# mfathulkr/MA-CJD-Cooperative-Jamming-Decision-Making-via-MARL

Measured on AMD Instinct MI355X. Metric: env-steps/sec (all GPUs; batch_envs=4096/GPU, 3j/4r), higher is better.
Workload: dtype f64; 1 GPU; 3 jammers / 4 radars, batch_envs=4096 per GPU, GRU hidden=64; mode=train, hidden=64, train_batch_episodes=32, updates_per_graph=20, hip_graphs=True, gemm_tuning=True, replay_capacity_episodes=8192, mixer_dtype=fp32, mixer=one MFMA launch per direction (f32)

## Files before the change

### include/macjd_nets.h

```cpp
#ifndef MACJD_NETS_H
#define MACJD_NETS_H

#include <stdint.h>

#include "macjd.h"

#ifdef __cplusplus
extern "C" {
#endif

typedef struct macjd_qhead_io {
    int64_t n_rows;
    int32_t H, A, n_agents, greedy_only;
    const float* base;  int64_t base_ld;
    const float* P_all; int64_t p_ld;
    const float* W1;    int64_t w1_ld;
    const float* w2;
    const float* b2;
    float* Q;           int64_t q_ld;
    const void* avail;  int32_t avail_elem_size, reserved;
    int64_t av_se, av_sj, av_sa;
    float epsilon;      float reserved2;
    uint64_t seed, counter;
    const float* eps_dev;
// ... 106 lines not shown
typedef struct macjd_wgrad_norm_io {
    int32_t ln_problem, partials_cap;
    const float* W; int64_t w_ld;
    float* dgamma; float* dbeta;
    float* partials;
    float* step;
} macjd_wgrad_norm_io;

int32_t macjd_linear_wgrad_many_norm_partials(const macjd_wgrad_io* ios, int32_t n, int32_t ln_problem);
int macjd_linear_wgrad_many_norm(const macjd_wgrad_io* ios, int32_t n, const macjd_wgrad_norm_io* norm, void* hip_stream);

int macjd_clip_adam_step_reduced(const macjd_adam_io* io, int32_t n_partials, const macjd_sampler_io* next, void* hip_stream);

typedef struct macjd_gather_io {
    int32_t n_tensors, n_rows;
    const int64_t* idx;
    const void* src[8]; void* dst[8]; int64_t row_bytes[8];
    int64_t dst_row_bytes[8];
} macjd_gather_io;

int macjd_gather_rows(const macjd_gather_io* io, void* hip_stream);

typedef struct macjd_prefetch_io {
    macjd_gru_io gru;
    macjd_gather_io gather;
    macjd_sampler_io sampler;
    macjd_tdloss_io mask;
    float* tot_m;
    int32_t no_draw, gather_blocks;
} macjd_prefetch_io;

int macjd_prefetch_batch_supported(int32_t n_nets, int32_t H, int32_t B);
int macjd_prefetch_batch(const macjd_prefetch_io* io, void* hip_stream);

typedef struct macjd_qinput_io {
    int64_t n_rows;
    int32_t H, A;
    const float* h;   int64_t h_ld;
    const void* idx;  int32_t idx_elem_size, reserved;
    const float* P;
    float* out;       int64_t out_ld;
} macjd_qinput_io;

int macjd_qhead_input(const macjd_qinput_io* io, void* hip_stream);

typedef struct macjd_qtaken_io {
    int64_t n_rows;
    int32_t H, A;
    const float* h;   int64_t h_ld;
    const void* idx;  int32_t idx_elem_size, reserved;
    const float* P;
    const float* W1;  int64_t w1_ld;
    const float* b1;  const float* w2;  const float* b2;
    float* x;         int64_t x_ld;
    float* act;       int64_t act_ld;
    float* q;
} macjd_qtaken_io;

int macjd_qhead_taken_supported(int32_t H, int32_t A);
int macjd_qhead_taken(const macjd_qtaken_io* io, void* hip_stream);

typedef struct macjd_layernorm_io {
    int64_t M;
    int32_t S, reserved;
    float eps, reserved2;
    const float* x;  int64_t x_ld;
// ... 238 lines not shown
```

### ma-cjd-cooperative-jamming-decision-making-via-marl_amd/_native.py

```python
from __future__ import annotations

import ctypes
import os
from typing import Optional

_PKG_DIR = os.path.dirname(os.path.abspath(__file__))
LIB_NAME = "libmacjd_hip.so"
LIB_PATH = os.environ.get("MACJD_LIB") or os.path.join(_PKG_DIR, LIB_NAME)

ABI_VERSION = 9
STEP_ARITH_F64 = 1
STEP_LANE_KERNEL = 2
STEP_SLOT_KERNEL = 4

EXPORTS = [
    "macjd_abi_version", "macjd_last_error", "macjd_reload_options", "macjd_device_count",
    "macjd_scenario_create", "macjd_scenario_destroy", "macjd_scenario_dims", "macjd_scenario_is_regular",
    "macjd_env_reset", "macjd_env_step", "macjd_env_step_timed",
    "macjd_qhead_select", "macjd_gru_sequence", "macjd_mixer_tail_forward", "macjd_mixer_tail_backward",
    "macjd_mlp_forward", "macjd_mlp_forward_pair", "macjd_td_loss", "macjd_clip_adam_step", "macjd_clip_adam_step_sample", "macjd_clip_adam_step_ln", "macjd_sample_episodes", "macjd_gather_rows",
    "macjd_linear_wgrad", "macjd_linear_wgrad_workspace_floats", "macjd_linear_wgrad_many", "macjd_qhead_input", "macjd_layernorm_forward", "macjd_layernorm_param_grad", "macjd_gru_gates", "macjd_rowdot", "macjd_splitrelu_backward",
    "macjd_mixer_fused_supported", "macjd_mixer_fused_forward", "macjd_mixer_fused_backward", "macjd_mixer_fused_backward_td", "macjd_td_mask_sum",
    "macjd_agent_episode_supported", "macjd_agent_episode", "macjd_env_step_many", "macjd_env_step_many_timed",
    "macjd_qhead_double_q_supported", "macjd_qhead_double_q", "macjd_qhead_taken_supported", "macjd_qhead_taken",
    "macjd_qheads_pair", "macjd_mixer_fused_forward_pair", "macjd_mixer_fused_train", "macjd_mixer_fused_train_static",
    "macjd_scenario_set_scan", "macjd_env_step_scan", "macjd_env_reset_scan",
    "macjd_env_step_scan_pe", "macjd_env_reset_scan_pe",
    "macjd_agent_env_episode_scan_supported", "macjd_agent_env_episode_scan",
    "macjd_scenario_set_scan_pattern",
    "macjd_gru_sequence_backward_supported", "macjd_gru_sequence_backward",
    "macjd_prefetch_batch_supported", "macjd_prefetch_batch",
    "macjd_actor_gradient_supported", "macjd_actor_gradient",
    "macjd_linear_wgrad_many_norm", "macjd_linear_wgrad_many_norm_partials", "macjd_clip_adam_step_reduced",
]


class NativeLibraryError(RuntimeError):
    pass


class StepIO(ctypes.Structure):
    _fields_ = [
        ("n_envs", ctypes.c_int64), ("env_offset", ctypes.c_int64), ("seed", ctypes.c_uint64),
        ("flags", ctypes.c_uint32), ("reserved", ctypes.c_uint32),
        ("T", ctypes.c_void_p), ("T_se", ctypes.c_int64), ("T_sx", ctypes.c_int64),
        ("P32", ctypes.c_void_p), ("P64", ctypes.c_void_p), ("P_se", ctypes.c_int64), ("P_sx", ctypes.c_int64),
        ("u", ctypes.c_void_p), ("u_se", ctypes.c_int64), ("u_sx", ctypes.c_int64),
        ("episode", ctypes.c_void_p),
        ("track", ctypes.c_void_p), ("k_se", ctypes.c_int64), ("k_sx", ctypes.c_int64),
        ("step", ctypes.c_void_p),
        ("reward", ctypes.c_void_p), ("r_dpj", ctypes.c_void_p), ("terminated", ctypes.c_void_p),
        ("pd", ctypes.c_void_p), ("pd_se", ctypes.c_int64), ("pd_sx", ctypes.c_int64),
        ("snr_with", ctypes.c_void_p), ("sw_se", ctypes.c_int64), ("sw_sx", ctypes.c_int64),
        ("out64", ctypes.c_void_p), ("pd64", ctypes.c_void_p), ("snr64", ctypes.c_void_p),
        ("prj64", ctypes.c_void_p),
        ("pe_tables", ctypes.c_void_p), ("pe_flags", ctypes.c_void_p), ("pe_stride", ctypes.c_int64),
        ("pe_tile", ctypes.c_int32), ("reserved_pe", ctypes.c_int32),
        ("r_dpj_sum", ctypes.c_void_p),
    ]


class ScanDesc(ctypes.Structure):
    _fields_ = [
        ("n_radars", ctypes.c_int32), ("n_jammers", ctypes.c_int32),
        ("half_beam", ctypes.c_void_p), ("sweep", ctypes.c_void_p), ("sweep_mod", ctypes.c_void_p),
        ("full", ctypes.c_void_p), ("az0", ctypes.c_void_p), ("bear_tgt", ctypes.c_void_p), ("bear_jam", ctypes.c_void_p),
# ... 404 lines not shown
    lib.macjd_mixer_fused_forward_pair.restype = ctypes.c_int
    lib.macjd_mixer_fused_forward_pair.argtypes = [ctypes.POINTER(MixerFusedIO), ctypes.POINTER(MixerFusedIO), ctypes.c_void_p]
    lib.macjd_qhead_input.restype = ctypes.c_int
    lib.macjd_qhead_input.argtypes = [ctypes.POINTER(QinputIO), ctypes.c_void_p]
    lib.macjd_layernorm_forward.restype = ctypes.c_int
    lib.macjd_layernorm_forward.argtypes = [ctypes.POINTER(LayerNormIO), ctypes.c_void_p]
    lib.macjd_gru_gates.restype = ctypes.c_int
    lib.macjd_gru_gates.argtypes = [ctypes.POINTER(GruGatesIO), ctypes.c_void_p]
    lib.macjd_splitrelu_backward.restype = ctypes.c_int
    lib.macjd_splitrelu_backward.argtypes = [ctypes.POINTER(SplitReluBwdIO), ctypes.c_void_p]
    lib.macjd_layernorm_param_grad.restype = ctypes.c_int
    lib.macjd_layernorm_param_grad.argtypes = [ctypes.POINTER(LnParamIO), ctypes.c_void_p]
    lib.macjd_rowdot.restype = ctypes.c_int
    lib.macjd_rowdot.argtypes = [ctypes.POINTER(RowdotIO), ctypes.c_void_p]
    lib.macjd_mlp_forward_pair.restype = ctypes.c_int
    lib.macjd_mlp_forward_pair.argtypes = [ctypes.POINTER(MlpIO), ctypes.POINTER(MlpIO), ctypes.c_void_p]
    lib.macjd_mlp_forward.restype = ctypes.c_int
    lib.macjd_mlp_forward.argtypes = [ctypes.POINTER(MlpIO), ctypes.c_void_p]
    lib.macjd_td_loss.restype = ctypes.c_int
    lib.macjd_td_loss.argtypes = [ctypes.POINTER(TdLossIO), ctypes.c_void_p]
    lib.macjd_clip_adam_step.restype = ctypes.c_int
    lib.macjd_clip_adam_step.argtypes = [ctypes.POINTER(AdamIO), ctypes.c_void_p]
    lib.macjd_clip_adam_step_sample.restype = ctypes.c_int
    lib.macjd_clip_adam_step_sample.argtypes = [ctypes.POINTER(AdamIO), ctypes.POINTER(SamplerIO), ctypes.c_void_p]
    lib.macjd_clip_adam_step_ln.restype = ctypes.c_int
    lib.macjd_clip_adam_step_ln.argtypes = [ctypes.POINTER(AdamIO), ctypes.POINTER(SamplerIO), ctypes.POINTER(LnParamIO),
                                            ctypes.c_int64, ctypes.c_int64, ctypes.c_void_p]
    lib.macjd_sample_episodes.restype = ctypes.c_int
    lib.macjd_sample_episodes.argtypes = [ctypes.POINTER(SamplerIO), ctypes.c_void_p]
    lib.macjd_prefetch_batch_supported.restype = ctypes.c_int
    lib.macjd_prefetch_batch_supported.argtypes = [ctypes.c_int32] * 3
    lib.macjd_prefetch_batch.restype = ctypes.c_int
    lib.macjd_prefetch_batch.argtypes = [ctypes.POINTER(PrefetchIO), ctypes.c_void_p]
    lib.macjd_gather_rows.restype = ctypes.c_int
    lib.macjd_gather_rows.argtypes = [ctypes.POINTER(GatherIO), ctypes.c_void_p]
    lib.macjd_linear_wgrad.restype = ctypes.c_int
    lib.macjd_linear_wgrad.argtypes = [ctypes.POINTER(WgradIO), ctypes.c_void_p]
    lib.macjd_linear_wgrad_many_norm.restype = ctypes.c_int
    lib.macjd_linear_wgrad_many_norm.argtypes = [ctypes.POINTER(WgradIO), ctypes.c_int32, ctypes.POINTER(WgradNormIO), ctypes.c_void_p]
    lib.macjd_linear_wgrad_many_norm_partials.restype = ctypes.c_int32
    lib.macjd_linear_wgrad_many_norm_partials.argtypes = [ctypes.POINTER(WgradIO), ctypes.c_int32, ctypes.c_int32]
    lib.macjd_clip_adam_step_reduced.restype = ctypes.c_int
    lib.macjd_clip_adam_step_reduced.argtypes = [ctypes.POINTER(AdamIO), ctypes.c_int32, ctypes.POINTER(SamplerIO), ctypes.c_void_p]
    lib.macjd_linear_wgrad_many.restype = ctypes.c_int
    lib.macjd_linear_wgrad_many.argtypes = [ctypes.POINTER(WgradIO), ctypes.c_int32, ctypes.c_void_p]
    lib.macjd_linear_wgrad_workspace_floats.restype = ctypes.c_int64
    lib.macjd_linear_wgrad_workspace_floats.argtypes = [ctypes.c_int64, ctypes.c_int32, ctypes.c_int32]
    if lib.macjd_abi_version() != ABI_VERSION:
        raise NativeLibraryError(f"{LIB_NAME}: ABI version {lib.macjd_abi_version()} != expected {ABI_VERSION}")
    _lib = lib
    return lib


def reload_options() -> None:
    load().macjd_reload_options()


def check(rc: int, what: str) -> None:
    if rc != 0:
        msg = load().macjd_last_error()
        raise NativeLibraryError(f"{what} failed ({rc}): {msg.decode() if msg else ''}")


class ScenarioHandle:

    def __init__(self, scenario):
# ... 31 lines not shown
```

### ma-cjd-cooperative-jamming-decision-making-via-marl_amd/core/qmix.py

```python
from __future__ import annotations

import copy
import os

import numpy as np
import torch
import torch.nn.functional as F
import torch.optim as optim

from .. import hipgraph, ops, options
from .networks import QMixer


def _to(x, dtype, device):
    if isinstance(x, torch.Tensor):
        return x.to(device=device, dtype=dtype)
    return torch.as_tensor(np.asarray(x), device=device).to(dtype)


class QMixLearner:
    def __init__(self, mac, args):
        self.args = args
        self.mac = mac
        self.n_agents = args.n_agents
        self.n_actions = args.n_actions
        self.state_shape = args.state_shape
        self.obs_shape = args.obs_shape
        self.device = torch.device(args.device if torch.cuda.is_available() and args.use_cuda else "cpu")
        self.train_agent_body = bool(getattr(args, "train_agent_body", False))
        self.train_actor = bool(getattr(args, "train_actor", False))
        self.actor_loss_coef = float(getattr(args, "actor_loss_coef", 1.0))
        self._last_actor_q = None

        self.eval_qmix_net = QMixer(args)
        self.target_mac = copy.deepcopy(mac)
        self.target_qmix_net = QMixer(args)
        self.target_qmix_net.load_state_dict(self.eval_qmix_net.state_dict())
        if args.use_cuda:
            self.cuda()
        print(f"QMix Learner Initialized on device: {self.device}")

        self.agent_params = list(self.mac.parameters())
        self.qmix_params = list(self.eval_qmix_net.parameters())
        self.params = self.agent_params + self.qmix_params
# ... 625 lines not shown
            with torch.no_grad():
                for p, sp in zip(self.params, snap_p):
                    p.copy_(sp)
                for p, st in self.optimizer.state.items():
                    for k, v in st.items():
                        if torch.is_tensor(v):
                            old = snap_o.get(id(p), {}).get(k)
                            v.copy_(old) if old is not None else v.zero_()
            if was_shared:
                self._mark_body_shared()

        restore_training_state()
        self._graph_a, self._graph_b = torch.cuda.CUDAGraph(), torch.cuda.CUDAGraph()
        self._g_graphed_ar = bool(graphed_allreduce if graphed_allreduce is not None
                                  else options.get("GRAPHED_ALLREDUCE") == "1") and self._ar_capturable()
        self._g_single = (self._world_size() <= 1 and not force_two_graphs) or self._g_graphed_ar
        with hipgraph.capture(self._graph_a):
            self._g_out_a = body_a()
            st4 = getattr(self, "_last_stats4", None) if fused else None
            if st4 is not None and st4.numel() == 4:
                self._grad_norm = st4[3]
            self._g_stats4 = st4 if (st4 is not None and st4.numel() == 4) else None
            nxt = (self._g_idx, self._g_n_stored, self._g_draws, self._sampler_seed()) if self._g_dev_sampler else None
            if self._g_single:
                if self._g_graphed_ar:
                    self._allreduce_grads(force=True)
                self._g_out_b = self._clip_and_step(sample_next=nxt)
        if not self._g_single:
            with hipgraph.capture(self._graph_b, pool=self._graph_a.pool()):
                self._g_out_b = self._clip_and_step(sample_next=nxt)
        K = int(updates_per_graph if updates_per_graph is not None else options.get("UPDATES_PER_GRAPH"))
        self._g_multi = None
        self._g_prefetch_launch = False
        if K > 1 and self._g_single and self._g_dev_sampler and fused and self._g_stats4 is not None:
            gm, rows, single_norm = torch.cuda.CUDAGraph(), [], self._grad_norm
            pipelined = (self._g_scan_from_ring and self._g_actor_in_scan and options.get("UPDATE_STREAMS") != "1"
                         and options.on("PIPELINED_GROUP"))
            launch_agents = [self.mac.agent] if self._body_is_shared() else [self.target_mac.agent, self.mac.agent]
            self._g_prefetch_launch = bool(pipelined and options.on("PREFETCH_LAUNCH") and "filled" in keys
                                           and ops.prefetch_batch_supported(launch_agents, self._g_B, srcs))
            stage2 = {k: torch.zeros_like(v) for k, v in stage.items()} if pipelined else None
            stages = [stage, stage2]
            self._g_stages = stages
            origin_dev = self.device

            unwritten = [0]

            def prefetch(dst, fork=True, draw=True):
                origin = torch.cuda.current_stream(origin_dev)
                ts = self._target_stream
                if isinstance(fork, torch.cuda.Event):
                    ts.wait_event(fork)
                elif fork:
                    ts.wait_stream(origin)
                shared = self._body_is_shared()
                agents = [self.mac.agent] if shared else [self.target_mac.agent, self.mac.agent]
                if self._g_prefetch_launch:
                    with torch.cuda.stream(ts), torch.no_grad():
                        h, ps, tot_m = ops.prefetch_batch(
                            buffer.buffers["obs"], agents, self._g_B, self.n_agents, self._g_T + 1,
                            (self._g_idx, self._g_n_stored, self._g_draws, self._sampler_seed()), srcs, [dst[k] for k in keys],
                            buffer.buffers["filled"], self._g_T - 1, offset=unwritten[0], draw=draw)
                        unwritten[0] += 1 if draw else 0
                        ev = torch.cuda.Event()
                        ev.record(ts)
                    return [h[0], h[0]], [ps[0], ps[0]], (ev, ev, tot_m)
                with torch.cuda.stream(ts), torch.no_grad():
                    if draw:
                        ops.sample_episodes(self._g_idx, self._g_n_stored, self._g_draws, self._sampler_seed())
                    ops.gather_rows(self._g_idx, srcs, [dst[k] for k in keys])
                    tot_m = ops.td_mask_sum(dst["filled"], self._g_T - 1)
                    ev_g = torch.cuda.Event()
                    ev_g.record(ts)
                    h, ps = ops.gru_sequence_from_obs(buffer.buffers["obs"], self._g_idx, agents, self._g_B, self.n_agents,
                                                      self._g_T + 1, with_actor=True)
                    ev_s = torch.cuda.Event()
                    ev_s.record(ts)
                return (([h[0], h[0]] if shared else h), ([ps[0], ps[0]] if shared else ps), (ev_g, ev_s, tot_m))

            with hipgraph.capture(gm, pool=self._graph_a.pool()):
                nxt_batch = None
                for k_upd in range(K):
                    last = k_upd == K - 1
                    box = {}
                    hook = (lambda fork=True: box.__setitem__("next", prefetch(stages[(k_upd + 1) % 2], fork))) if (pipelined and not last) else None
                    if pipelined and nxt_batch is not None:
                        h_pre, p_pre, evs = nxt_batch
                        self._forward_backward_full(stages[k_upd % 2], self._g_T, pre_scan=h_pre, pre_actor=p_pre,
                                                    prefetched=evs, after_join=hook)
                    elif pipelined:
                        pre = self._scan_from_ring_early()
                        ops.gather_rows(self._g_idx, srcs, [stage[k] for k in keys])
                        if self._paired_heads_ok(stage, self._g_T):
                            tot_m0 = ops.td_mask_sum(stage["filled"], self._g_T - 1)
                            scan_done = torch.cuda.Event()
                            scan_done.record(self._target_stream)
                            self._forward_backward_full(stage, self._g_T, pre_scan=pre[0], pre_actor=pre[1],
                                                        prefetched=(None, scan_done, tot_m0), after_join=hook)
                        else:
                            self._forward_backward_full(stage, self._g_T, pre_scan=pre[0], pre_actor=pre[1], after_join=hook)
                    else:
                        body_a()
                    nxt_batch = box.get("next")
                    rows.append(self._last_stats4)
                    self._grad_norm = rows[-1][3]
                    if self._g_graphed_ar:
                        self._allreduce_grads(force=True)
                    if nxt_batch is not None:
                        self._clip_and_step(sample_next=None)
                    else:
                        self._clip_and_step(sample_next=nxt + (unwritten[0],))
                        unwritten[0] = 0
                if pipelined:
                    torch.cuda.current_stream(self.device).wait_stream(self._target_stream)
            self._grad_norm = single_norm
            self._g_multi = (K, gm, rows)
            self._g_pipelined = pipelined
        self._g_shared_body = self._body_is_shared()
        assert self._g_obs_static == (bool(getattr(buffer, "obs_static", False)) and options.on("LEARNER_STATIC_OBS"))
        if prime:
            keep = (self._g_draws.clone(), self._g_idx.clone(), self._g_n_stored.clone())
            self._g_n_stored.fill_(int(buffer.current_size))
            self._g_idx.clamp_(0, max(0, int(buffer.current_size) - 1))
            hipgraph.replay(self._graph_a, self.device)
            if not self._g_single:
                self._allreduce_grads()
                hipgraph.replay(self._graph_b, self.device)
            if self._g_multi is not None:
                self._g_idx.clamp_(0, max(0, int(buffer.current_size) - 1))
                hipgraph.replay(self._g_multi[1], self.device)
            torch.cuda.synchronize(self.device)
            restore_training_state()
            self._g_draws.copy_(keep[0]); self._g_idx.copy_(keep[1]); self._g_n_stored.copy_(keep[2])
        self._graphs_ready = True

    def release_graphs(self):
        graphs = []
        m = getattr(self, "_g_multi", None)
        if m is not None:
            graphs.append(m[1])
        graphs += [getattr(self, "_graph_b", None), getattr(self, "_graph_a", None)]
        self._graphs_ready = False
        self._g_multi = self._g_stages = None
        self._graph_a = self._graph_b = None
        self._graph_body_a = None
        self._g_out_a = self._g_out_b = self._g_stats4 = self._last_stats4 = self._held_ln = self._norm_partials = None
        if self._flat_param is not None and any(g is not None for g in graphs):
            self._grad_norm = torch.zeros((), dtype=torch.float32, device=self._flat_param.device)
        hipgraph.destroy(graphs, self.device)

    def train_from_buffer(self, indices=None, sync_stats=True, stats_row=None):
        buf = self._g_buffer if getattr(self, "_graphs_ready", False) else None
        if buf is None:
            raise RuntimeError("call enable_graphs(buffer, batch_size) first")
        device_draw = False
        if indices is None:
            if buf.current_size < self._g_B:
                return self._snap(self.train(buf.sample(self._g_B), None, sync_stats=sync_stats), stats_row)
            device_draw = self._g_dev_sampler and self._population_full_length(buf)
            if not device_draw:
                indices = self._sample_rng.choice(buf.current_size, self._g_B, replace=False)
        if not device_draw:
            indices = np.asarray(indices, dtype=np.int64)
            if len(indices) != self._g_B or int(buf.episode_lengths[indices].min()) != self._g_T:
                return self._snap(self.train(buf.sample(len(indices), indices=indices), None, sync_stats=sync_stats), stats_row)
        if self._g_obs_static and not buf.obs_static:
            raise RuntimeError("an episode with unknown / changing observations was stored after enable_graphs() captured "
                               "the static-observation update: call enable_graphs() again")
        if self._g_shared_body and not self._body_is_shared():
            raise RuntimeError("the agent body (fc1 / GRU / actor) of one controller changed after enable_graphs() captured "
                               "the shared-body update: call enable_graphs() again")
        self.train_step += 1
        if device_draw:
            self._device_draw_ready(buf)
        else:
            k = self.train_step % len(self._g_idx_ring)
# ... 148 lines not shown
```

### ma-cjd-cooperative-jamming-decision-making-via-marl_amd/csrc/macjd_nets.hip

```cpp
#include <hip/hip_runtime.h>
#include <math.h>
#include <stdint.h>
#include <stdio.h>
#include <stdlib.h>
#include <string.h>
#include <type_traits>

#include "../../include/macjd.h"
#include "../../include/macjd_nets.h"
#include "macjd_err.h"
#include "macjd_tdloss.h"
#include "macjd_philox.h"
#include "macjd_gru_math.h"

namespace macjd {

static int set_nets_err(int code, const char* msg) { return set_err(code, "%s", msg); }

__device__ __forceinline__ bool avail_at(const macjd_qhead_io& io, int64_t e, int j, int a) {
    if (!io.avail) return true;
    const int64_t off = e * io.av_se + (int64_t)j * io.av_sj + (int64_t)a * io.av_sa;
    return (io.avail_elem_size == 8) ? (((const int64_t*)io.avail)[off] != 0)
                                     : (((const int32_t*)io.avail)[off] != 0);
}
// ... 855 lines not shown
        io.grad[i] = g;
        float m = io.exp_avg[i], v = io.exp_avg_sq[i];
        m = m + (1.0f - io.beta1) * (g - m);
        v = v * io.beta2 + (1.0f - io.beta2) * g * g;
        io.exp_avg[i] = m;
        io.exp_avg_sq[i] = v;
        const float denom = sqrtf(v) / bc2_sqrt + io.eps;
        io.param[i] -= step_size * (m / denom);
    }
    if (blockIdx.x == 0 && threadIdx.x == 0) io.grad_norm[0] = total_norm;
    if (SAMPLE && blockIdx.x == 0) sample_episodes_block(next);
}

template <bool SAMPLE>
__global__ void __launch_bounds__(256) adam_update_reduced_kernel(const macjd_adam_io io, const int n_partials, const macjd_sampler_io next) {
    __shared__ float s_w[4];
    float s = 0.0f;
    for (int base = 0; base < n_partials; base += 8 * 256) {
        float v[8];
#pragma unroll
        for (int j = 0; j < 8; ++j) {
            const int i = base + j * 256 + (int)threadIdx.x;
            v[j] = io.partials[i < n_partials ? i : n_partials - 1];
        }
#pragma unroll
        for (int j = 0; j < 8; ++j) s += (base + j * 256 + (int)threadIdx.x < n_partials) ? v[j] : 0.0f;
    }
    s = wave_sum(s);
    if ((threadIdx.x & 63) == 0) s_w[threadIdx.x >> 6] = s;
    __syncthreads();
    adam_apply<SAMPLE>(io, sqrtf((s_w[0] + s_w[1]) + (s_w[2] + s_w[3])), next);
}

__device__ __forceinline__ void gather_rows_body(const macjd_gather_io& io, const int k, const int row, const int64_t src_row,
                                                 const int part, const int parts) {
    const int64_t words = io.row_bytes[k] >> 2;
    const uint32_t* __restrict__ src = (const uint32_t*)((const char*)io.src[k] + src_row * io.row_bytes[k]);
    const int64_t dpitch = io.dst_row_bytes[k] ? io.dst_row_bytes[k] : io.row_bytes[k];
    uint32_t* __restrict__ dst = (uint32_t*)((char*)io.dst[k] + (int64_t)row * dpitch);
    const bool vec = ((io.row_bytes[k] & 15) == 0) && ((dpitch & 15) == 0) && ((((uintptr_t)io.src[k]) & 15) == 0) &&
                     ((((uintptr_t)io.dst[k]) & 15) == 0);
    if (vec) {
        const int64_t n4 = words >> 2;
        for (int64_t i = (int64_t)part * blockDim.x + threadIdx.x; i < n4; i += (int64_t)parts * blockDim.x)
            ((uint4*)dst)[i] = ((const uint4*)src)[i];
    } else {
        for (int64_t i = (int64_t)part * blockDim.x + threadIdx.x; i < words; i += (int64_t)parts * blockDim.x)
            dst[i] = src[i];
    }
}

__global__ void __launch_bounds__(256) gather_rows_kernel(const macjd_gather_io io) {
    gather_rows_body(io, blockIdx.y, blockIdx.z, io.idx[blockIdx.z], blockIdx.x, gridDim.x);
}

constexpr int PREFETCH_MAX_B = 1024;
constexpr int PREFETCH_ROW_PARTS = 8;

__global__ void __launch_bounds__(256) prefetch_batch_kernel(const macjd_prefetch_io io) {
    __shared__ __attribute__((aligned(16))) float s_h[2][64];
    __shared__ float s_gi[3 * 64];
    __shared__ float s_pro[768];
    __shared__ int64_t s_idx[PREFETCH_MAX_B];
    __shared__ float s_w[16];
    const int B = io.gru.B, BJ = B * io.gru.J, G = io.gather_blocks;
    const int wg = blockIdx.x;
    const int64_t N = (int64_t)*io.sampler.n_stored;
    const bool draw = !io.no_draw && N >= 1;
    SamplerPerm perm = {};
    if (draw) perm = sampler_perm(*io.sampler.counter + (int64_t)io.sampler.reserved, io.sampler.seed, N);
    auto index_of = [&](int t) -> int64_t { return draw ? sampler_index(perm, N, io.sampler.n, t) : io.sampler.idx_out[t]; };
    if (wg < 2 * BJ) {
        const bool actor_only = wg >= BJ;
        const int seq = actor_only ? wg - BJ : wg;
        gru_units_body<true>(io.gru, 0, seq, index_of(seq / io.gru.J), actor_only, false, s_h, s_gi, s_pro);
    } else if (wg < 2 * BJ + G) {
        const int n_parts = PREFETCH_ROW_PARTS * io.gather.n_tensors * B;
        for (int v = wg - 2 * BJ; v < n_parts; v += G) {
            const int part = v % PREFETCH_ROW_PARTS, kr = v / PREFETCH_ROW_PARTS;
            const int k = kr % io.gather.n_tensors, row = kr / io.gather.n_tensors;
            gather_rows_body(io.gather, k, row, index_of(row), part, PREFETCH_ROW_PARTS);
        }
    } else {
        for (int t = threadIdx.x; t < B; t += blockDim.x) {
            const int64_t e = index_of(t);
            s_idx[t] = e;
            if (draw) io.sampler.idx_out[t] = e;
        }
        __syncthreads();
        td_mask_sum_body(io.mask, io.tot_m, s_w, [&](int b) { return s_idx[b]; });
    }
}

}

static int sampler_args_ok(const macjd_sampler_io* sp) {
    return sp && sp->idx_out && sp->n >= 1 && sp->n_stored && sp->counter && sp->reserved >= 0;
}

extern "C" int macjd_sample_episodes(const macjd_sampler_io* io, void* hip_stream) {
    using namespace macjd;
    if (!sampler_args_ok(io)) return set_nets_err(MACJD_EINVAL, "macjd_sample_episodes: bad argument");
    hipLaunchKernelGGL(sample_episodes_kernel, dim3(1), dim3(256), 0, (hipStream_t)hip_stream, *io);
    hipError_t err = hipGetLastError();
    if (err != hipSuccess) return set_nets_err(MACJD_EDEVICE, hipGetErrorString(err));
    return MACJD_OK;
}

extern "C" int macjd_clip_adam_step_sample(const macjd_adam_io* io, const macjd_sampler_io* next, void* hip_stream) {
    using namespace macjd;
    if (!io || io->n < 1 || !io->param || !io->grad || !io->exp_avg || !io->exp_avg_sq || !io->step || !io->grad_norm ||
        !io->partials)
        return set_nets_err(MACJD_EINVAL, "macjd_clip_adam_step: bad argument");
    if (next && !sampler_args_ok(next)) return set_nets_err(MACJD_EINVAL, "macjd_clip_adam_step_sample: bad sampler argument");
    hipStream_t s = (hipStream_t)hip_stream;
    int blocks = (int)((io->n + 255) / 256);
    if (blocks > ADAM_BLOCKS) blocks = ADAM_BLOCKS;
    hipLaunchKernelGGL(adam_sqnorm_kernel, dim3(blocks), dim3(256), 0, s, *io);
    if (next) hipLaunchKernelGGL(adam_update_kernel<true>, dim3(blocks), dim3(256), 0, s, *io, blocks, *next);
    else hipLaunchKernelGGL(adam_update_kernel<false>, dim3(blocks), dim3(256), 0, s, *io, blocks, macjd_sampler_io{});
    hipError_t err = hipGetLastError();
    if (err != hipSuccess) return set_nets_err(MACJD_EDEVICE, hipGetErrorString(err));
    return MACJD_OK;
// ... 38 lines not shown
    if (next) hipLaunchKernelGGL(adam_update_kernel<true>, dim3(blocks), dim3(256), 0, s, *io, blocks + ln->K, *next);
    else hipLaunchKernelGGL(adam_update_kernel<false>, dim3(blocks), dim3(256), 0, s, *io, blocks + ln->K, macjd_sampler_io{});
    hipError_t err = hipGetLastError();
    if (err != hipSuccess) return set_nets_err(MACJD_EDEVICE, hipGetErrorString(err));
    return MACJD_OK;
}

static int gather_tensors_ok(const macjd_gather_io* io) {
    if (io->n_tensors < 1 || io->n_tensors > 8) return 0;
    for (int k = 0; k < io->n_tensors; ++k)
        if (!io->src[k] || !io->dst[k] || io->row_bytes[k] < 4 || (io->row_bytes[k] & 3) || (io->dst_row_bytes[k] & 3) ||
            (io->dst_row_bytes[k] && io->dst_row_bytes[k] < io->row_bytes[k]))
            return 0;
    return 1;
}

extern "C" int macjd_gather_rows(const macjd_gather_io* io, void* hip_stream) {
    using namespace macjd;
    if (!io || io->n_tensors < 1 || io->n_tensors > 8 || io->n_rows < 0 || !io->idx)
        return set_nets_err(MACJD_EINVAL, "macjd_gather_rows: bad argument");
    if (!gather_tensors_ok(io))
        return set_nets_err(MACJD_EINVAL, "macjd_gather_rows: bad tensor (row bytes must be a positive multiple of 4)");
    if (io->n_rows == 0) return MACJD_OK;
    hipLaunchKernelGGL(gather_rows_kernel, dim3(8, io->n_tensors, io->n_rows), dim3(256), 0, (hipStream_t)hip_stream, *io);
    hipError_t err = hipGetLastError();
    if (err != hipSuccess) return set_nets_err(MACJD_EDEVICE, hipGetErrorString(err));
    return MACJD_OK;
}

extern "C" int macjd_prefetch_batch_supported(int32_t n_nets, int32_t H, int32_t B) {
    return n_nets == 1 && H == 64 && B >= 1 && B <= macjd::PREFETCH_MAX_B && !macjd::env_options().gru_ksplit;
}

extern "C" int macjd_prefetch_batch(const macjd_prefetch_io* io, void* hip_stream) {
    using namespace macjd;
    if (!io) return set_nets_err(MACJD_EINVAL, "macjd_prefetch_batch: NULL io");
    const macjd_gru_io& g = io->gru;
    if (!macjd_prefetch_batch_supported(g.n_nets, g.H, g.B))
        return set_nets_err(MACJD_EUNSUPPORTED, "macjd_prefetch_batch: needs one network, H = 64, 1 <= B <= 1024, the unit-split scan");
    if (g.T < 1 || g.J < 1 || !g.obs || g.S < 1 || g.S > 256 || !g.w_hh[0] || !g.b_hh[0] || !g.h_out[0] || !g.fc1_w[0] ||
        !g.fc1_b[0] || !g.w_ih[0] || !g.b_ih[0])
        return set_nets_err(MACJD_EINVAL, "macjd_prefetch_batch: bad scan argument");
    if (!g.p_out[0] || g.Ah < 1 || g.Ah > 256 || g.A < 1 || g.A > 64)
        return set_nets_err(MACJD_EINVAL, "macjd_prefetch_batch: needs the in-kernel actor (Ah <= 256, A <= 64)");
    for (int l = 0; l < 3; ++l)
        if (!g.act_w[0][l] || !g.act_b[0][l]) return set_nets_err(MACJD_EINVAL, "macjd_prefetch_batch: needs the actor's three layers");
    if (!sampler_args_ok(&io->sampler) || io->sampler.n != g.B)
        return set_nets_err(MACJD_EINVAL, "macjd_prefetch_batch: bad sampler argument (n must be the batch size)");
    if (io->gather.n_rows != g.B || !gather_tensors_ok(&io->gather))
        return set_nets_err(MACJD_EINVAL, "macjd_prefetch_batch: bad gather argument (n_rows must be the batch size, row bytes "
                                          "positive multiples of 4)");
    if (io->mask.B != g.B || io->mask.Tm1 < 1 || !io->mask.filled || !io->tot_m)
        return set_nets_err(MACJD_EINVAL, "macjd_prefetch_batch: bad mask-sum argument");
    if (io->gather_blocks < 0) return set_nets_err(MACJD_EINVAL, "macjd_prefetch_batch: bad gather_blocks");
    macjd_prefetch_io a = *io;
    const int n_parts = PREFETCH_ROW_PARTS * a.gather.n_tensors * g.B;
    if (a.gather_blocks == 0) a.gather_blocks = 256;
    if (a.gather_blocks > n_parts) a.gather_blocks = n_parts;
    const unsigned grid = 2u * (unsigned)(g.B * g.J) + (unsigned)a.gather_blocks + 1u;
    hipLaunchKernelGGL(prefetch_batch_kernel, dim3(grid), dim3(256), 0, (hipStream_t)hip_stream, a);
    hipError_t err = hipGetLastError();
    if (err != hipSuccess) return set_nets_err(MACJD_EDEVICE, hipGetErrorString(err));
    return MACJD_OK;
}

namespace macjd {

__global__ void __launch_bounds__(256) qhead_input_kernel(const macjd_qinput_io io) {
    const int W = io.H + io.A + 1;
    const int64_t total = io.n_rows * W;
    for (int64_t i = (int64_t)blockIdx.x * blockDim.x + threadIdx.x; i < total; i += (int64_t)gridDim.x * blockDim.x) {
        const int64_t n = i / W;
        const int c = (int)(i - n * W);
        float v;
        if (c < io.H) {
            v = io.h[n * io.h_ld + c];
        } else if (c < io.H + io.A) {
            const int64_t a = (io.idx_elem_size == 8) ? ((const int64_t*)io.idx)[n] : (int64_t)((const int32_t*)io.idx)[n];
            v = (a == (int64_t)(c - io.H)) ? 1.0f : 0.0f;
        } else {
            v = io.P[n];
        }
        io.out[n * io.out_ld + c] = v;
    }
}

__global__ void __launch_bounds__(256) layernorm_forward_kernel(const macjd_layernorm_io io) {
    const int lane = threadIdx.x & 63;
    const int64_t wave = (int64_t)blockIdx.x * (blockDim.x >> 6) + (threadIdx.x >> 6);
    const int64_t n_waves = (int64_t)gridDim.x * (blockDim.x >> 6);
    const int S = io.S;
    const float inv_s = 1.0f / (float)S;
    for (int64_t m = wave; m < io.M; m += n_waves) {
        const float* __restrict__ x = io.x + m * io.x_ld;
        float v[16];
        float sum = 0.0f;
// ... 276 lines not shown
```

### ma-cjd-cooperative-jamming-decision-making-via-marl_amd/ops.py

```python
from __future__ import annotations

import ctypes
import os
from typing import Optional, Tuple

import numpy as np
import torch
import torch.nn.functional as F

from . import _native, options


def _stream(t: torch.Tensor) -> int:
    return torch.cuda.current_stream(t.device).cuda_stream


def _f32c(t: torch.Tensor) -> torch.Tensor:
    if t.dtype != torch.float32:
        t = t.float()
    return t if t.stride(-1) == 1 else t.contiguous()


def _qhead_fill(io: _native.QheadIO, base, P_all, W1, w2, b2, H: int, A: int, n_agents: int):
    io.n_rows, io.H, io.A, io.n_agents = base.shape[0], H, A, n_agents
# ... 1104 lines not shown


def gather_rows(idx, srcs, dsts):
    lib = _native.load()
    io = _gather_io(idx.numel(), srcs, dsts)
    io.idx = idx.data_ptr()
    with torch.cuda.device(idx.device):
        _native.check(lib.macjd_gather_rows(ctypes.byref(io), _stream(idx)), "macjd_gather_rows")


def prefetch_batch_supported(agents, B: int, srcs) -> bool:
    return (len(agents) == 1 and gather_rows_supported(srcs)
            and bool(_native.load().macjd_prefetch_batch_supported(len(agents), int(agents[0].rnn_hidden_dim), int(B))))


def prefetch_batch(obs, agents, B: int, J: int, n_steps: int, sampler, srcs, dsts, filled, Tm1: int, offset: int = 0,
                   draw: bool = True, gather_blocks: int = 0):
    lib = _native.load()
    if not prefetch_batch_supported(agents, B, srcs):
        raise _native.NativeLibraryError("macjd_prefetch_batch: unsupported shape (one agent body, rnn_hidden_dim 64, B <= 1024)")
    gio, outs, pouts, _keep = _gru_from_obs_io(obs, None, agents, B, J, n_steps, True)
    assert sampler[0].numel() == B and filled.dtype == torch.bool and filled.device == obs.device and filled.shape[1] >= Tm1
    io = _native.PrefetchIO()
    io.gru, io.gather, io.sampler = gio, _gather_io(B, srcs, dsts), _sampler_io(*sampler[:4], offset)
    io.mask.B, io.mask.Tm1 = int(B), int(Tm1)
    io.mask.filled, io.mask.f_sb, io.mask.f_st = filled.data_ptr(), filled.stride(0), filled.stride(1)
    tot_m = torch.empty(1, dtype=torch.float32, device=obs.device)
    io.tot_m, io.no_draw, io.gather_blocks = tot_m.data_ptr(), 0 if draw else 1, int(gather_blocks)
    with torch.cuda.device(obs.device):
        _native.check(lib.macjd_prefetch_batch(ctypes.byref(io), _stream(obs)), "macjd_prefetch_batch")
    return outs, pouts, tot_m


_DEFERRED_WGRAD = None
_DEFERRED_POST = None
_GRAD_DST = None
_DEFERRED_SEEN = None


def grad_key(t):
    return None if t is None else (t.data_ptr(), t.numel())


def _grad_dst(key, shape):
    if not _GRAD_DST or key is None:
        return None
    dst = _GRAD_DST.get(key)
    if dst is None or dst.numel() != int(np.prod(shape)) or not dst.is_contiguous():
        return None
    del _GRAD_DST[key]
    return dst.view(shape)


class deferred_wgrad:

    def __init__(self, grad_dst=None, hold_lnparam=False, norm=None):
        self._grad_dst = grad_dst
        self._hold, self.held = bool(hold_lnparam), []
        self._norm, self.norm_partials = norm, None

    def __enter__(self):
        global _DEFERRED_WGRAD, _DEFERRED_POST, _GRAD_DST, _DEFERRED_SEEN
        self._prev, _DEFERRED_WGRAD = _DEFERRED_WGRAD, []
        self._prev_post, _DEFERRED_POST = _DEFERRED_POST, []
        self._prev_dst, _GRAD_DST = _GRAD_DST, (dict(self._grad_dst) if self._grad_dst else None)
        self._prev_seen, _DEFERRED_SEEN = _DEFERRED_SEEN, set()
# ... 606 lines not shown
```

### ma-cjd-cooperative-jamming-decision-making-via-marl_amd/options.py

```python
from __future__ import annotations

import os

_DEFAULTS = {
    "UPDATE_STREAMS": "2", "UPDATES_PER_GRAPH": "1", "PIPELINED_GROUP": "1", "SHARED_BODY": "1",
    "LEARNER_STATIC_OBS": "1", "ACTOR_IN_SCAN": "1", "DEVICE_SAMPLER": "1", "LN_IN_SQNORM": "1", "NORM_IN_REDUCE": "1", "WGRAD_OUTER": "1",
    "QHEAD_TAKEN": "1", "QHEAD_DOUBLE_Q": "1", "QHEAD_DOUBLE_Q_H128": "0", "PAIRED_HEADS": "1", "MIXER_TRAIN": "1", "MIXER_STATIC_STATE": "1", "GRAPHED_ALLREDUCE": "0",
    "PREFETCH_LAUNCH": "1",
    "CLOSED_LOOP_ROLLOUT": "0",
}
_values = None


def reload() -> None:
    global _values
    _values = {k: os.environ.get("MACJD_" + k, d) for k, d in _DEFAULTS.items()}


def get(name: str) -> str:
    if _values is None:
        reload()
    return _values[name]


def on(name: str) -> bool:
    return get(name) != "0"
```

Measured before the change: 37.76 million env-steps/s.

## Prefetch two replay batches per fused launch in the multi-update graph

Extends the fused prefetch kernel so one launch can sample, gather and GRU-scan up to four replay batches, each with its own output slots. The captured multi-update graph now issues one prefetch launch every two updates, two updates ahead, using four rotating staging buffers. The goal is to halve the number of prefetch launches and give the side stream more lead time to overlap with the learner. The cost is more staging memory and a larger grid per launch that may contend with the main-stream work.

```diff
diff --git a/include/macjd_nets.h b/include/macjd_nets.h
--- a/include/macjd_nets.h
+++ b/include/macjd_nets.h
@@ -162,6 +162,10 @@
 
 int macjd_prefetch_batch_supported(int32_t n_nets, int32_t H, int32_t B);
 int macjd_prefetch_batch(const macjd_prefetch_io* io, void* hip_stream);
+
+#define MACJD_PREFETCH_MAX_BATCHES 4
+int macjd_prefetch_batches_supported(int32_t n_nets, int32_t H, int32_t B, int32_t n);
+int macjd_prefetch_batches(const macjd_prefetch_io* ios, int32_t n, void* hip_stream);
 
 typedef struct macjd_qinput_io {
     int64_t n_rows;
diff --git a/ma-cjd-cooperative-jamming-decision-making-via-marl_amd/_native.py b/ma-cjd-cooperative-jamming-decision-making-via-marl_amd/_native.py
--- a/ma-cjd-cooperative-jamming-decision-making-via-marl_amd/_native.py
+++ b/ma-cjd-cooperative-jamming-decision-making-via-marl_amd/_native.py
@@ -32,6 +32,7 @@
     "macjd_prefetch_batch_supported", "macjd_prefetch_batch",
     "macjd_actor_gradient_supported", "macjd_actor_gradient",
     "macjd_linear_wgrad_many_norm", "macjd_linear_wgrad_many_norm_partials", "macjd_clip_adam_step_reduced",
+    "macjd_prefetch_batches_supported", "macjd_prefetch_batches",
 ]
 
 
@@ -502,6 +503,10 @@
     lib.macjd_prefetch_batch_supported.argtypes = [ctypes.c_int32] * 3
     lib.macjd_prefetch_batch.restype = ctypes.c_int
     lib.macjd_prefetch_batch.argtypes = [ctypes.POINTER(PrefetchIO), ctypes.c_void_p]
+    lib.macjd_prefetch_batches_supported.restype = ctypes.c_int
+    lib.macjd_prefetch_batches_supported.argtypes = [ctypes.c_int32] * 4
+    lib.macjd_prefetch_batches.restype = ctypes.c_int
+    lib.macjd_prefetch_batches.argtypes = [ctypes.POINTER(PrefetchIO), ctypes.c_int32, ctypes.c_void_p]
     lib.macjd_gather_rows.restype = ctypes.c_int
     lib.macjd_gather_rows.argtypes = [ctypes.POINTER(GatherIO), ctypes.c_void_p]
     lib.macjd_linear_wgrad.restype = ctypes.c_int
diff --git a/ma-cjd-cooperative-jamming-decision-making-via-marl_amd/core/qmix.py b/ma-cjd-cooperative-jamming-decision-making-via-marl_amd/core/qmix.py
--- a/ma-cjd-cooperative-jamming-decision-making-via-marl_amd/core/qmix.py
+++ b/ma-cjd-cooperative-jamming-decision-making-via-marl_amd/core/qmix.py
@@ -1,5 +1,6 @@
 from __future__ import annotations
 
+import collections
 import copy
 import os
 
@@ -10,6 +11,21 @@
 
 from .. import hipgraph, ops, options
 from .networks import QMixer
+
+
+PrefetchLaunch = collections.namedtuple("PrefetchLaunch", "issue_at updates offsets sets")
+
+
+def prefetch_plan(K: int, ahead: int):
+    if ahead not in (1, 2):
+        raise ValueError("prefetch_plan: ahead must be 1 or 2")
+    n_sets = 2 * ahead
+    launches = []
+    for a in range(1, K, ahead):
+        updates = tuple(range(a, min(a + ahead, K)))
+        launches.append(PrefetchLaunch(max(0, a - ahead), updates, tuple(u - 1 for u in updates),
+                                       tuple(u % n_sets for u in updates)))
+    return launches, n_sets
 
 
 def _to(x, dtype, device):
@@ -701,6 +717,8 @@
         K = int(updates_per_graph if updates_per_graph is not None else options.get("UPDATES_PER_GRAPH"))
         self._g_multi = None
         self._g_prefetch_launch = False
+        self._g_prefetch_ahead = 1
+        self._g_prefetch_held = None
         if K > 1 and self._g_single and self._g_dev_sampler and fused and self._g_stats4 is not None:
             gm, rows, single_norm = torch.cuda.CUDAGraph(), [], self._grad_norm
             pipelined = (self._g_scan_from_ring and self._g_actor_in_scan and options.get("UPDATE_STREAMS") != "1"
@@ -708,8 +726,12 @@
             launch_agents = [self.mac.agent] if self._body_is_shared() else [self.target_mac.agent, self.mac.agent]
             self._g_prefetch_launch = bool(pipelined and options.on("PREFETCH_LAUNCH") and "filled" in keys
                                            and ops.prefetch_batch_supported(launch_agents, self._g_B, srcs))
-            stage2 = {k: torch.zeros_like(v) for k, v in stage.items()} if pipelined else None
-            stages = [stage, stage2]
+            plan = None
+            if self._g_prefetch_launch and options.get("PREFETCH_AHEAD") != "1":
+                plan, n_sets = prefetch_plan(K, 2)
+            self._g_prefetch_ahead = 2 if plan is not None else 1
+            stages = [stage] + ([{k: torch.zeros_like(v) for k, v in stage.items()} for _ in range(n_sets - 1 if plan else 1)]
+                                if pipelined else [None])
             self._g_stages = stages
             origin_dev = self.device
 
@@ -747,13 +769,49 @@
                     ev_s.record(ts)
                 return (([h[0], h[0]] if shared else h), ([ps[0], ps[0]] if shared else ps), (ev_g, ev_s, tot_m))
 
+            ready = {}
+            issues = {l.issue_at: l for l in plan} if plan is not None else {}
+            idx_rows = (torch.zeros(len(stages), self._g_B, dtype=torch.int64, device=self.device) if plan is not None else None)
+            self._g_prefetch_held = [idx_rows]
+            paired = plan is not None and self._paired_heads_ok(stage, self._g_T)
+
+            def prefetch_many(launch, fork=True):
+                origin = torch.cuda.current_stream(origin_dev)
+                ts = self._target_stream
+                if isinstance(fork, torch.cuda.Event):
+                    ts.wait_event(fork)
+                elif fork:
+                    ts.wait_stream(origin)
+                assert launch.offsets[0] == unwritten[0] and self._body_is_shared()
+                with torch.cuda.stream(ts), torch.no_grad():
+                    res = ops.prefetch_batches(
+                        buffer.buffers["obs"], [self.mac.agent], self._g_B, self.n_agents, self._g_T + 1,
+                        (self._g_n_stored, self._g_draws, self._sampler_seed()), srcs,
+                        [(off, True, [stages[s][k] for k in keys], idx_rows[s]) for off, s in zip(launch.offsets, launch.sets)],
+                        buffer.buffers["filled"], self._g_T - 1)
+                    unwritten[0] += len(launch.updates)
+                    ev = torch.cuda.Event()
+                    ev.record(ts)
+                self._g_prefetch_held.append(res)
+                for i, (u, (h, p, tot_m)) in enumerate(zip(launch.updates, res)):
+                    e = ev if (i == 0 or not paired) else None
+                    ready[u] = ([h, h], [p, p], (e, e, tot_m))
+
             with hipgraph.capture(gm, pool=self._graph_a.pool()):
                 nxt_batch = None
                 for k_upd in range(K):
                     last = k_upd == K - 1
                     box = {}
                     hook = (lambda fork=True: box.__setitem__("next", prefetch(stages[(k_upd + 1) % 2], fork))) if (pipelined and not last) else None
-                    if pipelined and nxt_batch is not None:
+                    if plan is not None:
+                        launch = issues.get(k_upd)
+                        hook = (lambda fork=True, launch=launch: prefetch_many(launch, fork)) if launch is not None else None
+                        nxt_batch = ready.pop(k_upd, None)
+                    if plan is not None and nxt_batch is not None:
+                        h_pre, p_pre, evs = nxt_batch
+                        self._forward_backward_full(stages[k_upd % len(stages)], self._g_T, pre_scan=h_pre, pre_actor=p_pre,
+                                                    prefetched=evs, after_join=hook)
+                    elif pipelined and nxt_batch is not None:
                         h_pre, p_pre, evs = nxt_batch
                         self._forward_backward_full(stages[k_upd % 2], self._g_T, pre_scan=h_pre, pre_actor=p_pre,
                                                     prefetched=evs, after_join=hook)
@@ -775,7 +833,7 @@
                     self._grad_norm = rows[-1][3]
                     if self._g_graphed_ar:
                         self._allreduce_grads(force=True)
-                    if nxt_batch is not None:
+                    if nxt_batch is not None or (plan is not None and not last):
                         self._clip_and_step(sample_next=None)
                     else:
                         self._clip_and_step(sample_next=nxt + (unwritten[0],))
@@ -810,7 +868,7 @@
             graphs.append(m[1])
         graphs += [getattr(self, "_graph_b", None), getattr(self, "_graph_a", None)]
         self._graphs_ready = False
-        self._g_multi = self._g_stages = None
+        self._g_multi = self._g_stages = self._g_prefetch_held = None
         self._graph_a = self._graph_b = None
         self._graph_body_a = None
         self._g_out_a = self._g_out_b = self._g_stats4 = self._last_stats4 = self._held_ln = self._norm_partials = None
diff --git a/ma-cjd-cooperative-jamming-decision-making-via-marl_amd/csrc/macjd_nets.hip b/ma-cjd-cooperative-jamming-decision-making-via-marl_amd/csrc/macjd_nets.hip
--- a/ma-cjd-cooperative-jamming-decision-making-via-marl_amd/csrc/macjd_nets.hip
+++ b/ma-cjd-cooperative-jamming-decision-making-via-marl_amd/csrc/macjd_nets.hip
@@ -911,14 +911,15 @@
     adam_apply<SAMPLE>(io, sqrtf((s_w[0] + s_w[1]) + (s_w[2] + s_w[3])), next);
 }
 
-__device__ __forceinline__ void gather_rows_body(const macjd_gather_io& io, const int k, const int row, const int64_t src_row,
-                                                 const int part, const int parts) {
+__device__ __forceinline__ void gather_rows_body(const macjd_gather_io& io, void* const dst_base, const int64_t dst_row_bytes,
+                                                 const int k, const int row, const int64_t src_row, const int part,
+                                                 const int parts) {
     const int64_t words = io.row_bytes[k] >> 2;
     const uint32_t* __restrict__ src = (const uint32_t*)((const char*)io.src[k] + src_row * io.row_bytes[k]);
-    const int64_t dpitch = io.dst_row_bytes[k] ? io.dst_row_bytes[k] : io.row_bytes[k];
-    uint32_t* __restrict__ dst = (uint32_t*)((char*)io.dst[k] + (int64_t)row * dpitch);
+    const int64_t dpitch = dst_row_bytes ? dst_row_bytes : io.row_bytes[k];
+    uint32_t* __restrict__ dst = (uint32_t*)((char*)dst_base + (int64_t)row * dpitch);
     const bool vec = ((io.row_bytes[k] & 15) == 0) && ((dpitch & 15) == 0) && ((((uintptr_t)io.src[k]) & 15) == 0) &&
-                     ((((uintptr_t)io.dst[k]) & 15) == 0);
+                     ((((uintptr_t)dst_base) & 15) == 0);
     if (vec) {
         const int64_t n4 = words >> 2;
         for (int64_t i = (int64_t)part * blockDim.x + threadIdx.x; i < n4; i += (int64_t)parts * blockDim.x)
@@ -930,44 +931,67 @@
 }
 
 __global__ void __launch_bounds__(256) gather_rows_kernel(const macjd_gather_io io) {
-    gather_rows_body(io, blockIdx.y, blockIdx.z, io.idx[blockIdx.z], blockIdx.x, gridDim.x);
+    gather_rows_body(io, io.dst[blockIdx.y], io.dst_row_bytes[blockIdx.y], blockIdx.y, blockIdx.z, io.idx[blockIdx.z], blockIdx.x,
+                     gridDim.x);
 }
 
 constexpr int PREFETCH_MAX_B = 1024;
 constexpr int PREFETCH_ROW_PARTS = 8;
 
-__global__ void __launch_bounds__(256) prefetch_batch_kernel(const macjd_prefetch_io io) {
+struct PrefetchSlot {
+    int64_t* idx_out;
+    float* h_out; float* p_out;
+    float* tot_m;
+    void* dst[8]; int64_t dst_row_bytes[8];
+    int32_t offset, no_draw;
+};
+struct PrefetchArgs {
+    macjd_prefetch_io sh;
+    int32_t n, reserved;
+    PrefetchSlot slot[MACJD_PREFETCH_MAX_BATCHES];
+};
+static_assert(sizeof(PrefetchArgs) <= 4096, "prefetch_batch_kernel: kernel arguments");
+
+__global__ void __launch_bounds__(256) prefetch_batch_kernel(const PrefetchArgs a) {
     __shared__ __attribute__((aligned(16))) float s_h[2][64];
     __shared__ float s_gi[3 * 64];
     __shared__ float s_pro[768];
     __shared__ int64_t s_idx[PREFETCH_MAX_B];
     __shared__ float s_w[16];
-    const int B = io.gru.B, BJ = B * io.gru.J, G = io.gather_blocks;
+    const int B = a.sh.gru.B, BJ = B * a.sh.gru.J, G = a.sh.gather_blocks, n = a.n;
     const int wg = blockIdx.x;
-    const int64_t N = (int64_t)*io.sampler.n_stored;
-    const bool draw = !io.no_draw && N >= 1;
+    const int r0 = n * BJ, r1 = 2 * r0, r2 = r1 + n * G;
+    const int share = wg < r1 ? BJ : (wg < r2 ? G : 1);
+    const int in_range = wg < r0 ? wg : (wg < r1 ? wg - r0 : (wg < r2 ? wg - r1 : wg - r2));
+    const int bi = in_range / share, local = in_range - bi * share;
+    const PrefetchSlot& sl = a.slot[bi];
+    const int64_t N = (int64_t)*a.sh.sampler.n_stored;
+    const bool draw = !sl.no_draw && N >= 1;
+    int64_t* const idx_out = sl.idx_out;
     SamplerPerm perm = {};
-    if (draw) perm = sampler_perm(*io.sampler.counter + (int64_t)io.sampler.reserved, io.sampler.seed, N);
-    auto index_of = [&](int t) -> int64_t { return draw ? sampler_index(perm, N, io.sampler.n, t) : io.sampler.idx_out[t]; };
-    if (wg < 2 * BJ) {
-        const bool actor_only = wg >= BJ;
-        const int seq = actor_only ? wg - BJ : wg;
-        gru_units_body<true>(io.gru, 0, seq, index_of(seq / io.gru.J), actor_only, false, s_h, s_gi, s_pro);
-    } else if (wg < 2 * BJ + G) {
-        const int n_parts = PREFETCH_ROW_PARTS * io.gather.n_tensors * B;
-        for (int v = wg - 2 * BJ; v < n_parts; v += G) {
+    if (draw) perm = sampler_perm(*a.sh.sampler.counter + (int64_t)sl.offset, a.sh.sampler.seed, N);
+    auto index_of = [&](int t) -> int64_t { return draw ? sampler_index(perm, N, a.sh.sampler.n, t) : idx_out[t]; };
+    if (wg < r1) {
+        const bool actor_only = wg >= r0;
+        macjd_gru_io g = a.sh.gru;
+        g.h_out[0] = sl.h_out;
+        g.p_out[0] = sl.p_out;
+        gru_units_body<true>(g, 0, local, index_of(local / g.J), actor_only, false, s_h, s_gi, s_pro);
+    } else if (wg < r2) {
+        const int n_parts = PREFETCH_ROW_PARTS * a.sh.gather.n_tensors * B;
+        for (int v = local; v < n_parts; v += G) {
             const int part = v % PREFETCH_ROW_PARTS, kr = v / PREFETCH_ROW_PARTS;
-            const int k = kr % io.gather.n_tensors, row = kr / io.gather.n_tensors;
-            gather_rows_body(io.gather, k, row, index_of(row), part, PREFETCH_ROW_PARTS);
+            const int k = kr % a.sh.gather.n_tensors, row = kr / a.sh.gather.n_tensors;
+            gather_rows_body(a.sh.gather, sl.dst[k], sl.dst_row_bytes[k], k, row, index_of(row), part, PREFETCH_ROW_PARTS);
         }
     } else {
         for (int t = threadIdx.x; t < B; t += blockDim.x) {
             const int64_t e = index_of(t);
             s_idx[t] = e;
-            if (draw) io.sampler.idx_out[t] = e;
+            if (draw) idx_out[t] = e;
         }
         __syncthreads();
-        td_mask_sum_body(io.mask, io.tot_m, s_w, [&](int b) { return s_idx[b]; });
+        td_mask_sum_body(a.sh.mask, sl.tot_m, s_w, [&](int b) { return s_idx[b]; });
     }
 }
 
@@ -1072,9 +1096,38 @@
     return n_nets == 1 && H == 64 && B >= 1 && B <= macjd::PREFETCH_MAX_B && !macjd::env_options().gru_ksplit;
 }
 
-extern "C" int macjd_prefetch_batch(const macjd_prefetch_io* io, void* hip_stream) {
-    using namespace macjd;
-    if (!io) return set_nets_err(MACJD_EINVAL, "macjd_prefetch_batch: NULL io");
+extern "C" int macjd_prefetch_batches_supported(int32_t n_nets, int32_t H, int32_t B, int32_t n) {
+    return n >= 1 && n <= MACJD_PREFETCH_MAX_BATCHES && macjd_prefetch_batch_supported(n_nets, H, B);
+}
+
+static int prefetch_shares_with_first(const macjd_prefetch_io* first, const macjd_prefetch_io* io) {
+    macjd_gru_io g = io->gru;
+    g.h_out[0] = first->gru.h_out[0];
+    g.p_out[0] = first->gru.p_out[0];
+    if (memcmp(&g, &first->gru, sizeof(g)) != 0) return 0;
+    macjd_sampler_io sp = io->sampler;
+    sp.idx_out = first->sampler.idx_out;
+    sp.reserved = first->sampler.reserved;
+    if (memcmp(&sp, &first->sampler, sizeof(sp)) != 0) return 0;
+    if (memcmp(&io->mask, &first->mask, sizeof(io->mask)) != 0) return 0;
+    if (io->gather.n_tensors != first->gather.n_tensors || io->gather.n_rows != first->gather.n_rows ||
+        io->gather_blocks != first->gather_blocks)
+        return 0;
+    for (int k = 0; k < first->gather.n_tensors; ++k)
+        if (io->gather.src[k] != first->gather.src[k] || io->gather.row_bytes[k] != first->gather.row_bytes[k]) return 0;
+    return 1;
+}
+
+static int prefetch_outputs_distinct(const macjd_prefetch_io* x, const macjd_prefetch_io* y) {
+    if (x->gru.h_out[0] == y->gru.h_out[0] || x->gru.p_out[0] == y->gru.p_out[0] || x->tot_m == y->tot_m) return 0;
+    if (x->sampler.idx_out == y->sampler.idx_out && !(x->no_draw && y->no_draw)) return 0;
+    for (int k = 0; k < x->gather.n_tensors; ++k)
+        if (x->gather.dst[k] == y->gather.dst[k]) return 0;
+    return 1;
+}
+
+static int prefetch_one_ok(const macjd_prefetch_io* io) {
+    using namespace macjd;
     const macjd_gru_io& g = io->gru;
     if (!macjd_prefetch_batch_supported(g.n_nets, g.H, g.B))
         return set_nets_err(MACJD_EUNSUPPORTED, "macjd_prefetch_batch: needs one network, H = 64, 1 <= B <= 1024, the unit-split scan");
@@ -1093,15 +1146,53 @@
     if (io->mask.B != g.B || io->mask.Tm1 < 1 || !io->mask.filled || !io->tot_m)
         return set_nets_err(MACJD_EINVAL, "macjd_prefetch_batch: bad mask-sum argument");
     if (io->gather_blocks < 0) return set_nets_err(MACJD_EINVAL, "macjd_prefetch_batch: bad gather_blocks");
-    macjd_prefetch_io a = *io;
-    const int n_parts = PREFETCH_ROW_PARTS * a.gather.n_tensors * g.B;
-    if (a.gather_blocks == 0) a.gather_blocks = 256;
-    if (a.gather_blocks > n_parts) a.gather_blocks = n_parts;
-    const unsigned grid = 2u * (unsigned)(g.B * g.J) + (unsigned)a.gather_blocks + 1u;
+    return MACJD_OK;
+}
+
+extern "C" int macjd_prefetch_batches(const macjd_prefetch_io* ios, int32_t n, void* hip_stream) {
+    using namespace macjd;
+    if (!ios) return set_nets_err(MACJD_EINVAL, "macjd_prefetch_batch: NULL io");
+    if (n < 1 || n > MACJD_PREFETCH_MAX_BATCHES)
+        return set_nets_err(MACJD_EINVAL, "macjd_prefetch_batches: 1 <= n <= MACJD_PREFETCH_MAX_BATCHES");
+    for (int i = 0; i < n; ++i) {
+        const int rc = prefetch_one_ok(&ios[i]);
+        if (rc != MACJD_OK) return rc;
+        if (i > 0 && !prefetch_shares_with_first(&ios[0], &ios[i]))
+            return set_nets_err(MACJD_EINVAL, "macjd_prefetch_batches: the batches of a launch differ only in the counter offset, no_draw, "
+                                              "idx_out, gather.dst / dst_row_bytes, h_out, p_out and tot_m");
+        for (int j = 0; j < i; ++j)
+            if (!prefetch_outputs_distinct(&ios[j], &ios[i]))
+                return set_nets_err(MACJD_EINVAL, "macjd_prefetch_batches: two batches share an output");
+    }
+    PrefetchArgs a = {};
+    a.sh = ios[0];
+    a.n = n;
+    for (int i = 0; i < n; ++i) {
+        PrefetchSlot& sl = a.slot[i];
+        sl.idx_out = ios[i].sampler.idx_out;
+        sl.h_out = ios[i].gru.h_out[0];
+        sl.p_out = ios[i].gru.p_out[0];
+        sl.tot_m = ios[i].tot_m;
+        for (int k = 0; k < ios[i].gather.n_tensors; ++k) {
+            sl.dst[k] = ios[i].gather.dst[k];
+            sl.dst_row_bytes[k] = ios[i].gather.dst_row_bytes[k];
+        }
+        sl.offset = ios[i].sampler.reserved;
+        sl.no_draw = ios[i].no_draw;
+    }
+    const macjd_gru_io& g = a.sh.gru;
+    const int n_parts = PREFETCH_ROW_PARTS * a.sh.gather.n_tensors * g.B;
+    if (a.sh.gather_blocks == 0) a.sh.gather_blocks = 256;
+    if (a.sh.gather_blocks > n_parts) a.sh.gather_blocks = n_parts;
+    const unsigned grid = (unsigned)n * (2u * (unsigned)(g.B * g.J) + (unsigned)a.sh.gather_blocks + 1u);
     hipLaunchKernelGGL(prefetch_batch_kernel, dim3(grid), dim3(256), 0, (hipStream_t)hip_stream, a);
     hipError_t err = hipGetLastError();
     if (err != hipSuccess) return set_nets_err(MACJD_EDEVICE, hipGetErrorString(err));
     return MACJD_OK;
+}
+
+extern "C" int macjd_prefetch_batch(const macjd_prefetch_io* io, void* hip_stream) {
+    return macjd_prefetch_batches(io, 1, hip_stream);
 }
 
 namespace macjd {
diff --git a/ma-cjd-cooperative-jamming-decision-making-via-marl_amd/ops.py b/ma-cjd-cooperative-jamming-decision-making-via-marl_amd/ops.py
--- a/ma-cjd-cooperative-jamming-decision-making-via-marl_amd/ops.py
+++ b/ma-cjd-cooperative-jamming-decision-making-via-marl_amd/ops.py
@@ -1160,6 +1160,38 @@
     return outs, pouts, tot_m
 
 
+PREFETCH_MAX_BATCHES = 4
+
+
+def prefetch_batches(obs, agents, B: int, J: int, n_steps: int, sampler, srcs, batches, filled, Tm1: int,
+                     gather_blocks: int = 0):
+    lib = _native.load()
+    n = len(batches)
+    if not (1 <= n <= PREFETCH_MAX_BATCHES and prefetch_batch_supported(agents, B, srcs)
+            and lib.macjd_prefetch_batches_supported(len(agents), int(agents[0].rnn_hidden_dim), int(B), n)):
+        raise _native.NativeLibraryError("macjd_prefetch_batches: unsupported shape (1 to 4 batches, one agent body, "
+                                         "rnn_hidden_dim 64, B <= 1024)")
+    n_stored, counter, seed = sampler
+    assert filled.dtype == torch.bool and filled.device == obs.device and filled.shape[1] >= Tm1
+    gio, outs, pouts, _keep = _gru_from_obs_io(obs, None, agents, B, J, n_steps, True)
+    ios, res = (_native.PrefetchIO * n)(), []
+    for i, (offset, draw, dsts, idx_out) in enumerate(batches):
+        assert idx_out.numel() == B
+        io = ios[i]
+        io.gru = gio
+        h, p = (outs[0], pouts[0]) if i == 0 else (torch.empty_like(outs[0]), torch.empty_like(pouts[0]))
+        io.gru.h_out[0], io.gru.p_out[0] = h.data_ptr(), p.data_ptr()
+        io.gather, io.sampler = _gather_io(B, srcs, dsts), _sampler_io(idx_out, n_stored, counter, seed, offset)
+        io.mask.B, io.mask.Tm1 = int(B), int(Tm1)
+        io.mask.filled, io.mask.f_sb, io.mask.f_st = filled.data_ptr(), filled.stride(0), filled.stride(1)
+        tot_m = torch.empty(1, dtype=torch.float32, device=obs.device)
+        io.tot_m, io.no_draw, io.gather_blocks = tot_m.data_ptr(), 0 if draw else 1, int(gather_blocks)
+        res.append((h, p, tot_m))
+    with torch.cuda.device(obs.device):
+        _native.check(lib.macjd_prefetch_batches(ios, n, _stream(obs)), "macjd_prefetch_batches")
+    return res
+
+
 _DEFERRED_WGRAD = None
 _DEFERRED_POST = None
 _GRAD_DST = None
diff --git a/ma-cjd-cooperative-jamming-decision-making-via-marl_amd/options.py b/ma-cjd-cooperative-jamming-decision-making-via-marl_amd/options.py
--- a/ma-cjd-cooperative-jamming-decision-making-via-marl_amd/options.py
+++ b/ma-cjd-cooperative-jamming-decision-making-via-marl_amd/options.py
@@ -6,7 +6,7 @@
     "UPDATE_STREAMS": "2", "UPDATES_PER_GRAPH": "1", "PIPELINED_GROUP": "1", "SHARED_BODY": "1",
     "LEARNER_STATIC_OBS": "1", "ACTOR_IN_SCAN": "1", "DEVICE_SAMPLER": "1", "LN_IN_SQNORM": "1", "NORM_IN_REDUCE": "1", "WGRAD_OUTER": "1",
     "QHEAD_TAKEN": "1", "QHEAD_DOUBLE_Q": "1", "QHEAD_DOUBLE_Q_H128": "0", "PAIRED_HEADS": "1", "MIXER_TRAIN": "1", "MIXER_STATIC_STATE": "1", "GRAPHED_ALLREDUCE": "0",
-    "PREFETCH_LAUNCH": "1",
+    "PREFETCH_LAUNCH": "1", "PREFETCH_AHEAD": "2",
     "CLOSED_LOOP_ROLLOUT": "0",
 }
 _values = None
```

Measured after the change: 39.82 million env-steps/s, median of 6. +5.5%, better.
